# IllyaArtemchuk/Harmonies-Alphazero

Measured on AMD Instinct MI355X. Metric: self-play env-steps/sec + games/sec @4096 boards, 1/2/4/8 GPUs; bit-exact vs CPU, higher is better.
Workload: dtype u64; 1 GPU; config2: 4096 concurrent boards/GPU, reset + rule-driven play to game end (legal mask, step, chance draws, final scoring); one step = 256 hz_play launches of 4096 boards; boards_per_gpu=4096, parallelism=shard1

## Files before the change

### harmonies-alphazero_amd/csrc/hz_net.hip

```cpp
#include <hip/hip_runtime.h>

#include <atomic>
#include <cstdint>
#include <cstdlib>
#include <type_traits>

#include "../../include/hz_abi.h"
#include "hz_host.hpp"

using namespace hz_host;

namespace {

template <bool Res>
__global__ void __launch_bounds__(256) k_bias_act(float4 *__restrict__ x, const float4 *__restrict__ bias,
                                                  const float4 *__restrict__ res, int64_t n4, int32_t ch4) {
  int64_t i = (int64_t)blockIdx.x * 256 + threadIdx.x;
  if (i >= n4) return;
  float4 v = x[i];
  float4 b = bias[(int32_t)(i % ch4)];
  v.x = v.x + b.x;
  v.y = v.y + b.y;
  v.z = v.z + b.z;
  v.w = v.w + b.w;
// ... 706 lines not shown
    }
  }
  HZ_STAMP(7)
  HZ_STAMP_RT(9)
}
#undef HZ_X6_LOAD
#undef HZ_X6_STORE
#undef HZ_X6_SYNC

}

#ifndef HZ_KO
#define HZ_KO 0
#endif
namespace {
constexpr int kW4Stg = (kRows * 8 + 255) / 256;

template <int B, int E, class F>
__device__ __forceinline__ void static_for(F &&f) {
  if constexpr (B < E) {
    f(std::integral_constant<int, B>{});
    static_for<B + 1, E>(f);
  }
}
constexpr int x6_class_blocks(int h, int tap) {
  int k = 0;
  for (int rb = 0; rb < 9; rb++) k += (kX6ClassTaps[h][rb] >> tap) & 1;
  return k;
}

template <bool Block, bool Cf = false>
// ... 6 lines not shown
  if constexpr (NT) return __builtin_nontemporal_load((const f32x4 *)p);
  return *(const f32x4 *)p;
}
template <bool NT>
__device__ __forceinline__ float4 x6_ld4f(const float *p) {
  if constexpr (NT) {
    const f32x4 v = __builtin_nontemporal_load((const f32x4 *)p);
    return make_float4(v[0], v[1], v[2], v[3]);
  }
  return *(const float4 *)p;
}
template <bool Tower>
using X6In = std::conditional_t<Tower, const float *, const float *__restrict__>;
template <bool Tower>
using X6Out = std::conditional_t<Tower, float *, float *__restrict__>;
template <bool Block, bool Cf, bool Tower>
__device__ __forceinline__ void x6w4_body(X6In<Tower> x, const bf16x8 *__restrict__ wp,
                                          const float *__restrict__ bias, X6In<Tower> res,
                                          X6Out<Tower> out, int32_t batch, const int32_t *__restrict__ live,
                                          const bf16x8 *__restrict__ wp2, const float *__restrict__ bias2,
                                          float *__restrict__ tmp) {
  constexpr int NQ = 4, kRBT = 9, NCB = 4, NG = Block ? 8 : 4;
  constexpr int kZero = kCS * 35 * kX6Cell;
  constexpr int kBufT = kZero + kX6Zero;
  constexpr int kE = 2 * kBufT;
  static_assert(kZero % 256 == 0, "zero region 256-B aligned");
  constexpr int kDummyCell = kE + (kRows + 1) * 128;
  static_assert(kDummyCell + kX6Cell <= 160 * 1024, "buffers, E and the dummy cell fit the LDS");
  extern __shared__ float4 lds4[];
  char *lds = (char *)lds4;
  int t0 = threadIdx.x;
  if constexpr (Tower) asm volatile("" : "+v"(t0));
  __builtin_assume(t0 >= 0 && t0 < 256);
  const int t = t0, lane = t & 63, w = t >> 6, kg = lane >> 4, rh = w >> 1, chf = w & 1;
  const int s0 = blockIdx.x * kCS;
  if (live) batch = *live < batch ? *live : batch;
  if (s0 >= batch) return;
  const int ns = batch - s0 < kCS ? batch - s0 : kCS;
  HZ_STAMP(0)
  HZ_STAMP_RT(8)

  if (t < 2 * kX6Zero / 16) {
    const int b = t / (kX6Zero / 16), k = t - b * (kX6Zero / 16);
    *(float4 *)(lds + b * kBufT + kZero + 16 * k) = make_float4(0.f, 0.f, 0.f, 0.f);
  }
  f32x4 stg[kW4Stg];
  auto stage_f = [&](int it) {
    const int f = it * 256 + t;
    return f < kRows * 8 ? f : kRows * 8 - 1;
  };
  auto srow = [](int f) {
    const int r = f >> 3;
    return (r & ~3) | ((r & 1) << 1) | ((r >> 1) & 1);
// ... 2 lines not shown
  auto opaque_t = [&]() __attribute__((always_inline)) {
    int tt = t;
    if constexpr (Block) asm volatile("" : "+v"(tt));
    return tt;
  };
  auto stage_issue = [&](int q) __attribute__((always_inline)) {
    const int tt = opaque_t();
#pragma unroll
    for (int it = 0; it < kW4Stg; it++) {
      int f = it * 256 + tt;
      f = f < kRows * 8 ? f : kRows * 8 - 1;
      const int sc = s0 * 35 + srow(f);
      stg[it] = x6_ld4<Tower>(x + (size_t)(sc < last_row ? sc : last_row) * 128 + 4 * (f & 7) + 32 * q);
    }
  };
  constexpr int kTmpRows = 288;
  float *const tmpg = Block ? tmp + (size_t)blockIdx.x * 2 * kTmpRows * 32 : nullptr;
  auto stage_issue_e = [&]() __attribute__((always_inline)) {
    const int tt = opaque_t();
#pragma unroll
    for (int it = 0; it < kW4Stg; it++) {
      int f = it * 256 + tt;
      f = f < kRows * 8 ? f : kRows * 8 - 1;
      stg[it] = *(const f32x4 *)(lds + kE + 128 * srow(f) + 16 * (f & 7));
    }
  };
  auto stage_issue_tmp = [&](int half) __attribute__((always_inline)) {
    const int tt = opaque_t();
#pragma unroll
    for (int it = 0; it < kW4Stg; it++) {
      int f = it * 256 + tt;
      f = f < kRows * 8 ? f : kRows * 8 - 1;
      stg[it] = x6_ld4<Tower>(tmpg + half * kTmpRows * 32 + 32 * srow(f) + 4 * (f & 7));
    }
  };
  auto stage_put = [&](int it, int buf) {
    uint2 h, m, l;
    split4(stg[it], h, m, l);
    const int f = stage_f(it);
    char *d = lds + buf * kBufT + srow(f) * kX6Cell + 8 * (f & 7);
    *(uint2 *)d = h;
    *(uint2 *)(d + 64) = m;
    *(uint2 *)(d + 128) = l;
  };
  const int co0 = 64 * chf + (lane & 15);
  const bf16x8 *wl = wp + co0 * 4 + kg;
  const bf16x8 *wl2 = (Block ? wp2 : wp) + co0 * 4 + kg;
  auto bissue = [&](bf16x8(&dst)[3][NCB], int S) {
    S = S < 9 * NG ? S : 9 * NG - 1;
    const bf16x8 *w = wl;
    if constexpr (Block) {
      w = S < 9 * NQ ? wl : wl2;
      S = S < 9 * NQ ? S : S - 9 * NQ;
    }
    const int q2 = S / 9, t2 = S - 9 * q2;
#pragma unroll
    for (int p = 0; p < 3; p++)
#pragma unroll
      for (int cb = 0; cb < NCB; cb++) dst[p][cb] = w[((t2 * NQ + q2) * 3 + p) * 512 + 64 * cb];
  };
  int rtab[kRBT];
#pragma unroll
  for (int rb = 0; rb < kRBT; rb++) rtab[rb] = x6_tab<Block, Cf>()[rh * kRBT + rb][lane & 15];
  stage_issue(0);
  bf16x8 b[3][NCB], bn[3][NCB];
  bissue(b, 0);

  int cbase[kRBT];
  uint32_t valid[kRBT];
#pragma unroll
  for (int rb = 0; rb < kRBT; rb++) {
    const int r = rtab[rb] >= 0 ? rtab[rb] : 0;
    const int s = r / 35, cell = r - 35 * s, ch = cell / 7, cw = cell - 7 * ch;
    uint32_t v = 0;
#pragma unroll
    for (int tap = 0; tap < 9; tap++) {
      const int hh = ch + tap / 3 - 1, ww = cw + tap % 3 - 1;
      v |= (uint32_t)(hh >= 0 && hh < 5 && ww >= 0 && ww < 7) << tap;
// ... 9 lines not shown

  f32x4 acc[kRBT][NCB];
#pragma unroll
  for (int rb = 0; rb < kRBT; rb++)
#pragma unroll
    for (int cb = 0; cb < NCB; cb++) acc[rb][cb] = (f32x4){};
  HZ_STAMP(1)
#pragma unroll
  for (int it = 0; it < kW4Stg; it++) stage_put(it, 0);
  __syncthreads();
  HZ_STAMP(2)

  auto switch_convs = [&]() __attribute__((always_inline)) {
    float b1v[NCB];
#pragma unroll
    for (int cb = 0; cb < NCB; cb++) b1v[cb] = bias[64 * chf + 16 * cb + (lane & 15)];
    uint2 rows[kRBT];
#pragma unroll
    for (int rb = 0; rb < kRBT; rb++) rows[rb] = *(const uint2 *)&x6_tab<Block, Cf>()[rh * kRBT + rb][4 * kg];
    auto put_all = [&](auto chfc) __attribute__((always_inline)) {
      constexpr int C = decltype(chfc)::value;
      static_for<0, kRBT>([&](auto rbc) {
        constexpr int rb = decltype(rbc)::value;
        static_for<0, 4>([&](auto jc) {
          constexpr int j = decltype(jc)::value;
          const int r = (int)(int16_t)((j < 2 ? rows[rb].x : rows[rb].y) >> (16 * (j & 1)));
          const bool pad = r < 0;
          static_for<0, NCB>([&](auto cbc) {
            constexpr int cb = decltype(cbc)::value;
            float v = acc[rb][cb][j] + b1v[cb];
            v = v > 0.f ? v : 0.f;
            const int k = 16 * (cb & 1) + (lane & 15);
            if constexpr (cb >= 2) {
              tmpg[C * kTmpRows * 32 + (pad ? kRows : r) * 32 + k] = v;
            } else if constexpr (C == 0) {
              const uint32_t h = bf16_bits(v);
              const float r1 = v - bf16_value(h);
              const uint32_t m = bf16_bits(r1);
              const uint32_t l = bf16_bits(r1 - bf16_value(m));
              char *d = lds + (pad ? kDummyCell : r * kX6Cell) + 2 * k;
              *(unsigned short *)d = (unsigned short)h;
              *(unsigned short *)(d + 64) = (unsigned short)m;
              *(unsigned short *)(d + 128) = (unsigned short)l;
            } else {
              *(float *)(lds + kE + (pad ? kRows : r) * 128 + 4 * k) = v;
            }
          });
        });
        static_for<0, NCB>([&](auto cbc) { acc[rb][decltype(cbc)::value] = (f32x4){}; });
      });
    };
    if (chf == 0)
      put_all(std::integral_constant<int, 0>{});
    else
      put_all(std::integral_constant<int, 1>{});
    __syncthreads();
  };
  auto classed = [&](auto half) {
    constexpr int H = decltype(half)::value;
    auto aread = [&](bf16x8(&dst)[kRBT], const char *lb, auto tapc, int pa) {
      constexpr int tap = decltype(tapc)::value;
      static_for<0, kRBT>([&](auto rbc) {
        constexpr int rb = decltype(rbc)::value;
        if constexpr ((kX6ClassTaps[H][rb] >> tap) & 1) {
          constexpr int kNeg = 8 * kX6Cell;
          const int d = ((tap / 3 - 1) * 7 + (tap % 3 - 1)) * kX6Cell + kNeg + 64 * pa;
          if constexpr ((kX6ClassSel[H][rb] >> tap) & 1)
            dst[rb] = *(const bf16x8 *)(lb + aoff(rb, tap) + 64 * pa);
          else
            dst[rb] = *(const bf16x8 *)(lb - kNeg + cbase[rb] + d);
// ... 30 lines not shown
            if (tap == 0 && stage && !(HZ_KO & 1)) {
              if (Block && g == NQ + 1)
                stage_issue_e();
              else if (Block && g >= NQ)
                stage_issue_tmp(g == NQ + 2);
              else
                stage_issue(q + 1);
            }
          }
          if constexpr (HZ_KO & 2) {
            if (tap == 7 && pa == 1 && stage)
#pragma unroll
              for (int it = 0; it < kW4Stg; it++) asm volatile("" ::"v"(stg[it]));
          } else if constexpr (pa == 1 && !(HZ_KO & 1)) {
            if (stage) {
              if constexpr (tap >= 2 && tap <= 4) {
                stage_put(2 * (tap - 2), nb);
                stage_put(2 * (tap - 2) + 1, nb);
              } else if constexpr (tap >= 5 && tap <= 7) {
                stage_put(tap + 1, nb);
              }
            }
          }
#pragma unroll
          for (int pb = 0; pb < 3 - pa; pb++)
            static_for<0, kRBT>([&](auto rbc) {
              constexpr int rb = decltype(rbc)::value;
              if constexpr ((kX6ClassTaps[H][rb] >> tap) & 1) {
#pragma unroll
                for (int cb = 0; cb < NCB; cb++)
                  acc[rb][cb] = __builtin_amdgcn_mfma_f32_16x16x32_bf16(a[(HZ_KO & 32) ? 0 : cur][rb], b[pb][cb],
// ... 10 lines not shown
#pragma unroll
          for (int p = 0; p < 3; p++)
#pragma unroll
            for (int cb = 0; cb < NCB; cb++) b[p][cb] = bn[p][cb];
        }
      });
      __builtin_amdgcn_sched_barrier(0);
      if (sync) __syncthreads();
      if (g < NQ) {
        HZ_STAMP(3 + g)
      } else {
        HZ_STAMP(7 + g)
      }
    }
  };
  if (rh == 0)
    classed(std::integral_constant<int, 0>{});
  else
    classed(std::integral_constant<int, 1>{});

  constexpr int kTS = 20, kT = 6;
  static_assert(4 * kT * 16 * kTS * 4 <= kZero, "per-wave tiles fit in buffer 0");
  float *tile = (float *)lds + w * 16 * kTS * kT;
  const int trow = lane >> 2, tcol = 4 * (lane & 3);
  const int cow = 64 * chf + tcol;
  const int nrow = ns * 35;
  const size_t gbase = (size_t)s0 * 35 * 128;
  int erow[kRBT];
#pragma unroll
  for (int rb = 0; rb < kRBT; rb++) erow[rb] = x6_tab<Block, Cf>()[rh * kRBT + rb][lane >> 2];
  auto orow = [&](int rb) -> int {
    const int row = erow[rb];
    return row >= 0 && row < nrow ? row : -1;
  };
  const float *eres = Block ? x : res, *ebias = Block ? bias2 : bias;
  float4 rv[kRBT * NCB];
#pragma unroll
  for (int k = 0; k < kRBT * NCB; k++) {
    const int rb = k / NCB, cb = k % NCB;
    const int row = orow(rb);
    rv[k] = eres && row >= 0 && !(HZ_KO & 64) ? x6_ld4f<Tower>(eres + gbase + (size_t)row * 128 + cow + 16 * cb)
                                              : make_float4(0.f, 0.f, 0.f, 0.f);
  }
  if constexpr (Tower) asm volatile("" ::: "memory");
  float4 bv[NCB];
// ... 38 lines not shown
          if (never) *(float4 *)(out + gbase + (size_t)row * 128 + cow + 16 * cb) = v;
        } else
          *(float4 *)(out + gbase + (size_t)row * 128 + cow + 16 * cb) = v;
      }
    }
  }
  HZ_STAMP(7)
  HZ_STAMP_RT(9)
}
template <bool Block, bool Cf = false>
__global__ void __launch_bounds__(256, 1)
    k_conv3x3_x6w4(const float *__restrict__ x, const bf16x8 *__restrict__ wp, const float *__restrict__ bias,
                   const float *__restrict__ res, float *__restrict__ out, int32_t batch,
                   const int32_t *__restrict__ live, const bf16x8 *__restrict__ wp2,
                   const float *__restrict__ bias2, float *__restrict__ tmp) {
  x6w4_body<Block, Cf, false>(x, wp, bias, res, out, batch, live, wp2, bias2, tmp);
}
constexpr int kTowerMax = 16;
struct X6Tower {
  const bf16x8 *w1[kTowerMax], *w2[kTowerMax];
  const float *b1[kTowerMax], *b2[kTowerMax];
  int32_t nblk;
  int32_t stagger;
  int32_t round;
};
template <bool Cf>
__global__ void __launch_bounds__(256, 1)
    k_x6w4_tower(const float *__restrict__ x, float *out, int32_t batch, const int32_t *__restrict__ live,
                 float *__restrict__ tmp, X6Tower tw) {
  if (tw.stagger > 0 && (int)blockIdx.x < tw.round && ((blockIdx.x >> 3) & 1))
    for (int i = 0; i < tw.stagger; i++) __builtin_amdgcn_s_sleep(127);
#pragma unroll 1
  for (int k = 0; k < tw.nblk; k++) {
    x6w4_body<true, Cf, true>(k == 0 ? x : out, tw.w1[k], tw.b1[k], nullptr, out, batch, live, tw.w2[k], tw.b2[k],
                              tmp);
    asm volatile("s_waitcnt vmcnt(0)" ::: "memory");
    __syncthreads();
  }
}
}
#undef HZ_STAMP
#undef HZ_STAMP_RT

template <int NQ, bool Stem, int CS, int NCB, int Ord = 2>
static int launch_x6_cs(const float *x, const void *wpack6, const float *bias, const float *res, float *out,
                        int32_t batch, const int32_t *live, void *stream) {
  const size_t lds = 2 * (size_t)((CS * 35 * kX6Cell + 255) / 256 * 256 + kX6Zero);
  if (lds_opt_in<k_conv3x3_x6<NQ, Stem, CS, NCB, Ord>>(lds)) return 1;
  hipLaunchKernelGGL((k_conv3x3_x6<NQ, Stem, CS, NCB, Ord>), dim3((batch + CS - 1) / CS),
                     dim3((CS == 8 ? 2 : 1) * (8 / NCB) * 64), lds, (hipStream_t)stream, x, (const bf16x8 *)wpack6,
// ... 15 lines not shown
  static const bool v = env_pick("HZ_X6_W4", 0, 1);
  return v;
}

template <bool Block, bool Cf = false>
static int launch_x6w4(const float *x, const void *wpack6, const float *bias, const float *res, float *out,
                       int32_t batch, const int32_t *live, void *stream, const void *wpack6_2 = nullptr,
                       const float *bias2 = nullptr, float *tmp = nullptr) {
  const size_t lds = 2 * (size_t)(kCS * 35 * kX6Cell + kX6Zero) + (Block ? (size_t)(kRows + 1) * 128 + kX6Cell : 0);
  if (lds_opt_in<k_conv3x3_x6w4<Block, Cf>>(lds)) return 1;
  hipLaunchKernelGGL((k_conv3x3_x6w4<Block, Cf>), dim3((batch + kCS - 1) / kCS), dim3(256), lds, (hipStream_t)stream, x,
                     (const bf16x8 *)wpack6, bias, res, out, batch, live, (const bf16x8 *)wpack6_2, bias2, tmp);
  return hipGetLastError() == hipSuccess ? 0 : 1;
}

template <bool Cf>
static int launch_x6w4_tower(const float *x, float *out, float *tmp, const X6Tower &tw, int32_t batch,
                             const int32_t *live, void *stream) {
  const size_t lds = 2 * (size_t)(kCS * 35 * kX6Cell + kX6Zero) + (size_t)(kRows + 1) * 128 + kX6Cell;
  if (lds_opt_in<k_x6w4_tower<Cf>>(lds)) return 1;
  hipLaunchKernelGGL((k_x6w4_tower<Cf>), dim3((batch + kCS - 1) / kCS), dim3(256), lds, (hipStream_t)stream, x, out,
                     batch, live, tmp, tw);
  return hipGetLastError() == hipSuccess ? 0 : 1;
}

static Setting g_x6_block{"HZ_X6_BLOCK", 1};
static bool x6_block() { return g_x6_block.get() != 0; }

static Setting g_x6_blk_cf{"HZ_BLK_TABLE", 1};
static bool x6_blk_cf() { return g_x6_blk_cf.get() != 0; }

static bool stem_cs4() {
  static const bool v = env_pick("HZ_STEM_CS4", 0, 1);
  return v;
}
static bool x6_cs4() {
// ... 65 lines not shown
    int dev = 0, n = 0;
    if (hipGetDevice(&dev) == hipSuccess &&
        hipDeviceGetAttribute(&n, hipDeviceAttributeMultiprocessorCount, dev) == hipSuccess && n > 0)
      v = n;
    else
      v = 256;
    cus.store(v, std::memory_order_relaxed);
  }
  return v;
}
extern "C" int hz_tower_x6_set_stagger(int32_t units) {
  if (units < 0 || units > 1000) return -1;
  g_tower_stagger.set(units);
  return 0;
}
extern "C" int hz_tower_x6_blocks(const float *x, const void *const *w1, const float *const *b1,
                                  const void *const *w2, const float *const *b2, int32_t nblk, float *out,
                                  float *tmp, int32_t batch, const int32_t *live, void *stream) {
  if (!x || !w1 || !b1 || !w2 || !b2 || !out || !tmp || batch < 0 || nblk < 1 || nblk > kTowerMax) return -1;
  if (((uintptr_t)x | (uintptr_t)out | (uintptr_t)tmp) & 15) return -1;
  if (batch == 0) return 0;
  if (!hz_resblock_x6_fused(batch)) return -2;
  X6Tower tw{};
  for (int k = 0; k < nblk; k++) {
    if (!w1[k] || !b1[k] || !w2[k] || !b2[k] || (((uintptr_t)w1[k] | (uintptr_t)w2[k]) & 15)) return -1;
    tw.w1[k] = (const bf16x8 *)w1[k];
    tw.w2[k] = (const bf16x8 *)w2[k];
    tw.b1[k] = b1[k];
    tw.b2[k] = b2[k];
  }
  tw.nblk = nblk;
  tw.stagger = g_tower_stagger.get();
  tw.round = tower_round();
  return x6_blk_cf() ? launch_x6w4_tower<true>(x, out, tmp, tw, batch, live, stream)
                     : launch_x6w4_tower<false>(x, out, tmp, tw, batch, live, stream);
}

extern "C" int hz_resblock_x6_set_fused(int32_t on) {
  if (on != 0 && on != 1) return -1;
  g_x6_block.set(on);
  return 0;
}

extern "C" int hz_resblock_x6_set_table(int32_t cf) {
  if (cf != 0 && cf != 1) return -1;
  g_x6_blk_cf.set(cf);
  return 0;
}
// ... 14 lines not shown
namespace {
constexpr int kTRZero = 31 * 256;
constexpr int kTRChunk = kTRZero + 256 + 256;
constexpr int kTRBuf = 4 * kTRChunk;
constexpr int kTRLds = 2 * kTRBuf + 35 * 128 * 4;
constexpr int kTRMaxConv = 64;
constexpr int kTRConvW = 9 * 4 * 3 * 128 * 4;
constexpr int kTRAhead = 4;
static_assert(35 * kX6Cell <= kTRZero && kTRZero + 255 + 128 + 16 <= kTRChunk, "cells and zero region fit");
static_assert(36 % kTRAhead == 0, "the B ring's slots repeat every conv");

template <int Ord = 2>
__global__ void __launch_bounds__(512, 1)
    k_tower_x6_resident(const float *__restrict__ x0, const bf16x8 *__restrict__ wp,
                        const float *__restrict__ bias, float *__restrict__ out, int32_t nconv, int32_t batch,
                        const int32_t *__restrict__ live) {
  extern __shared__ float4 lds4[];
  char *lds = (char *)lds4;
  float *skip = (float *)(lds + 2 * kTRBuf);
  float *biasl = skip + 35 * 128;
  const int t = threadIdx.x, lane = t & 63, w = t >> 6, kg = lane >> 4;
  const int s = blockIdx.x;
  if (live) batch = *live < batch ? *live : batch;
  if (s >= batch) return;
  for (int i = t; i < nconv * 128; i += 512) biasl[i] = bias[i];

  if (t < 2 * 4 * 32) {
    const int c = t >> 5, k = t & 31;
    *(float4 *)(lds + c * kTRChunk + kTRZero + 16 * k) = make_float4(0.f, 0.f, 0.f, 0.f);
  }
  const float *xs = x0 + (size_t)s * 35 * 128;
  for (int f = t; f < 35 * 32; f += 512) {
    const f32x4 v = *(const f32x4 *)(xs + 4 * f);
    const int cell = f >> 5, part = f & 31;
    uint2 h, m, l;
    split4(v, h, m, l);
    char *d = lds + (part >> 3) * kTRChunk + cell * kX6Cell + 8 * (part & 7);
    *(uint2 *)d = h;
    if constexpr (Ord >= 1) *(uint2 *)(d + 64) = m;
// ... 93 lines not shown
  }
  static_assert(kTRAhead == 4, "the final wait names the ring's four slots");
  if constexpr (Ord == 2)
    asm volatile("s_waitcnt vmcnt(0)" ::: "memory");
  else if constexpr (Ord == 1)
    asm volatile("s_waitcnt vmcnt(0)"
                 : "+v"(bq[0][0]), "+v"(bq[0][1]), "+v"(bq[1][0]), "+v"(bq[1][1]), "+v"(bq[2][0]), "+v"(bq[2][1]),
                   "+v"(bq[3][0]), "+v"(bq[3][1])
                 :
                 : "memory");
  else
    asm volatile("s_waitcnt vmcnt(0)" : "+v"(bq[0][0]), "+v"(bq[1][0]), "+v"(bq[2][0]), "+v"(bq[3][0]) : : "memory");
}
}

extern "C" int hz_tower_x6_resident(const float *x0, const void *wpack6, const float *bias, float *out,
                                    int32_t nconv, int32_t batch, const int32_t *live, void *stream) {
  if (!x0 || !wpack6 || !bias || !out || batch < 0 || nconv < 2 || nconv > kTRMaxConv || (nconv & 1)) return -1;
  if (((uintptr_t)x0 | (uintptr_t)wpack6 | (uintptr_t)out) & 15) return -1;
  if (batch == 0) return 0;
  if (lds_opt_in<k_tower_x6_resident<>>(kTRLds + kTRMaxConv * 128 * 4)) return 1;
  hipLaunchKernelGGL(k_tower_x6_resident<>, dim3(batch), dim3(512), kTRLds + nconv * 128 * 4, (hipStream_t)stream, x0,
                     (const bf16x8 *)wpack6, bias, out, nconv, batch, live);
  return hipGetLastError() == hipSuccess ? 0 : 1;
}

template <int Ord>
static int launch_resident_xn(const float *x0, const void *wpack6, const float *bias, float *out, int32_t nconv,
                              int32_t batch, const int32_t *live, void *stream) {
  if (lds_opt_in<k_tower_x6_resident<Ord>>(kTRLds + kTRMaxConv * 128 * 4)) return 1;
  hipLaunchKernelGGL(k_tower_x6_resident<Ord>, dim3(batch), dim3(512), kTRLds + nconv * 128 * 4, (hipStream_t)stream,
                     x0, (const bf16x8 *)wpack6, bias, out, nconv, batch, live);
  return hipGetLastError() == hipSuccess ? 0 : 1;
}

extern "C" int hz_tower_xn_resident(const float *x0, const void *wpack6, const float *bias, float *out,
                                    int32_t nconv, int32_t batch, const int32_t *live, int32_t products,
                                    void *stream) {
  if (products != 1 && products != 3 && products != 6) return -1;
  if (products == 6) return hz_tower_x6_resident(x0, wpack6, bias, out, nconv, batch, live, stream);
  if (!x0 || !wpack6 || !bias || !out || batch < 0 || nconv < 2 || nconv > kTRMaxConv || (nconv & 1)) return -1;
  if (((uintptr_t)x0 | (uintptr_t)wpack6 | (uintptr_t)out) & 15) return -1;
  if (batch == 0) return 0;
  return products == 3 ? launch_resident_xn<1>(x0, wpack6, bias, out, nconv, batch, live, stream)
                       : launch_resident_xn<0>(x0, wpack6, bias, out, nconv, batch, live, stream);
}

// ... 791 lines not shown
```

### harmonies-alphazero_amd/hzamd/_native.py

```python
import ctypes
import os

import torch

PKG_DIR = os.path.dirname(os.path.dirname(os.path.abspath(__file__)))
LIB_PATH = os.environ.get("HZ_LIB") or os.path.join(PKG_DIR, "libhz.so")

_lib = None

_c = ctypes
_vp = ctypes.c_void_p
_SIGS = {
    "hz_env_create": ([_c.c_int32, _c.c_uint64, _vp], _vp),
    "hz_env_destroy": ([_vp], None),
    "hz_env_size": ([_vp], _c.c_int32),
    "hz_env_set_stream": ([_vp, _vp], _c.c_int),
    "hz_env_state_ptr": ([_vp], _vp),
    "hz_env_mt_ptr": ([_vp], _vp),
    "hz_env_mt_pos_ptr": ([_vp], _vp),
    "hz_env_stream_ptrs": ([_vp, _vp, _vp, _vp], _c.c_int),
    "hz_env_ply_ptr": ([_vp], _vp),
    "hz_env_seed_ptr": ([_vp], _vp),
    "hz_reset": ([_vp, _vp, _vp], _c.c_int),
    "hz_legal_mask": ([_vp, _vp, _vp], _c.c_int),
# ... 53 lines not shown
    "hz_bias_act": ([_vp, _vp, _vp, _c.c_int64, _c.c_int32, _vp], _c.c_int),
    "hz_conv3x3_bias_act": ([_vp, _vp, _vp, _vp, _vp, _c.c_int32, _vp, _vp], _c.c_int),
    "hz_heads": ([_vp, _vp, _vp, _vp, _vp, _vp, _c.c_int32, _vp, _vp], _c.c_int),
    "hz_heads_fc": ([_vp] * 13 + [_c.c_int32, _vp, _vp], _c.c_int),
    "hz_conv3x3_x6_bias_act": ([_vp, _vp, _vp, _vp, _vp, _c.c_int32, _vp, _vp], _c.c_int),
    "hz_conv3x3_xn_bias_act": ([_vp, _vp, _vp, _vp, _vp, _c.c_int32, _vp, _c.c_int32, _vp], _c.c_int),
    "hz_tower_xn_resident": ([_vp, _vp, _vp, _vp, _c.c_int32, _c.c_int32, _vp, _c.c_int32, _vp], _c.c_int),
    "hz_stem3x3_x6_bias_act": ([_vp, _vp, _vp, _vp, _c.c_int32, _vp, _vp], _c.c_int),
    "hz_resblock_x6_bias_act": ([_vp, _vp, _vp, _vp, _vp, _vp, _vp, _c.c_int32, _vp, _vp], _c.c_int),
    "hz_resblock_x6_fused": ([_c.c_int32], _c.c_int32),
    "hz_resblock_x6_set_fused": ([_c.c_int32], _c.c_int),
    "hz_resblock_x6_set_table": ([_c.c_int32], _c.c_int),
    "hz_tower_x6_set_stagger": ([_c.c_int32], _c.c_int),
    "hz_tower_x6_blocks": ([_vp, _vp, _vp, _vp, _vp, _c.c_int32, _vp, _vp, _c.c_int32, _vp, _vp], _c.c_int),
    "hz_tower_x6_resident": ([_vp, _vp, _vp, _vp, _c.c_int32, _c.c_int32, _vp, _vp], _c.c_int),
    "hz_tower_x6_split": ([_vp, _vp, _vp, _vp, _vp, _vp, _c.c_int32, _c.c_int32, _vp, _vp], _c.c_int),
    "hz_tower_x6_split_max_batch": ([], _c.c_int32),
    "hz_tower_x6_split_set_limit": ([_c.c_int32], _c.c_int),
    "hz_conv3x3_x6g_bias_act": ([_vp, _vp, _vp, _vp, _vp, _c.c_int32, _c.c_int32, _c.c_int32, _vp, _c.c_int32,
                                 _c.c_int32, _vp], _c.c_int),
    "hz_stem3x3_x6g_bias_act": ([_vp, _vp, _vp, _vp, _c.c_int32, _c.c_int32, _vp, _c.c_int32, _vp], _c.c_int),
    "hz_heads_fc_g": ([_vp] * 13 + [_c.c_int32] * 5 + [_vp, _vp], _c.c_int),
    "hz_stem3x3_bias_act": ([_vp, _vp, _vp, _vp, _c.c_int32, _vp, _vp], _c.c_int),
    "hz_version": ([], _c.c_char_p),
}


class NativeError(RuntimeError):
    pass

# ... 41 lines not shown
```

### harmonies-alphazero_amd/hzamd/infer.py

```python
import ctypes
import os

import torch
import torch.nn.functional as F
from torch import nn

from ._native import NativeError, lib


def pack_conv3x3(w):
    co, ci = w.shape[0], w.shape[1]
    return w.permute(2, 3, 1, 0).reshape(9, ci // 16, 16, co).permute(0, 1, 3, 2).contiguous()


def split3_bf16(w):
    w = w.float()
    h = w.to(torch.bfloat16)
    r = w - h.float()
    m = r.to(torch.bfloat16)
    lo = (r - m.float()).to(torch.bfloat16)
    return torch.stack((h, m, lo))


def pack_conv3x3_x6(w):
# ... 189 lines not shown

def _resblock_x6(x, p1, b1, p2, b2, live=None):
    if not (x.is_cuda and x.dtype == torch.float32 and x.is_contiguous(memory_format=torch.channels_last)
            and x.shape[1:] == (128, 5, 7)):
        raise NativeError("hz_resblock_x6_bias_act needs a CUDA fp32 channels_last [B,128,5,7] activation")
    out = torch.empty_like(x, memory_format=torch.channels_last)
    tmp = torch.empty_like(x, memory_format=torch.channels_last)
    rc = lib().hz_resblock_x6_bias_act(x.data_ptr(), p1.data_ptr(), b1.data_ptr(), p2.data_ptr(), b2.data_ptr(),
                                       out.data_ptr(), tmp.data_ptr(), x.shape[0], _live_ptr(live),
                                       torch.cuda.current_stream(x.device).cuda_stream)
    if rc != 0:
        raise NativeError(f"hz_resblock_x6_bias_act failed ({rc})")
    return out


def _tower_blocks_x6(x, ptrs, nblk, live=None):
    out = torch.empty_like(x, memory_format=torch.channels_last)
    tmp = torch.empty_like(x, memory_format=torch.channels_last)
    w1, b1, w2, b2 = ptrs
    rc = lib().hz_tower_x6_blocks(x.data_ptr(), w1, b1, w2, b2, nblk, out.data_ptr(), tmp.data_ptr(), x.shape[0],
                                  _live_ptr(live), torch.cuda.current_stream(x.device).cuda_stream)
    if rc == -2:
        return None
    if rc != 0:
        raise NativeError(f"hz_tower_x6_blocks failed ({rc})")
    return out


def pack_stem_x6(w):
    co = w.shape[0]
    w64 = torch.zeros(co, 64, 3, 3, dtype=w.dtype, device=w.device)
    w64[:, :w.shape[1]] = w
    w64[:, 38] = w64[:, 39] = w[:, 37]
    pl = split3_bf16(w64)
    pl[2, :, 38] = 0
    pl[1:, :, 39] = 0
# ... 151 lines not shown
def _fold(conv, bn):
    inv = torch.rsqrt(bn.running_var.double() + bn.eps) * bn.weight.double()
    w = (conv.weight.double() * inv.view(-1, 1, 1, 1)).float()
    b0 = conv.bias.double() if conv.bias is not None else torch.zeros_like(inv)
    b = ((b0 - bn.running_mean.double()) * inv + bn.bias.double()).float()
    return w.contiguous(memory_format=torch.channels_last), b.contiguous()


class FoldedNet(nn.Module):

    TOWER_MFMA = ("x6", "x3", "x1", "f32")
    TOWER_PRODUCTS = {"x6": 6, "x3": 3, "x1": 1}
    resident_max = int(os.environ.get("HZ_RESIDENT_MAX", "896"))
    split_max = int(os.environ.get("HZ_SPLIT_MAX", "32"))
    tower_loop = int(os.environ.get("HZ_TOWER_LOOP", "1"))
    wide_spg = 0

    def __init__(self, net, epilogue=None, native_conv=True, tower=None, fused_head=True):
        super().__init__()
        if tower is None:
            tower = os.environ.get("HZ_TOWER", "x6")
        if tower not in self.TOWER_MFMA:
            raise ValueError(f"tower must be one of {self.TOWER_MFMA}, not {tower!r}")
        self.src = net
        self.tower = tower
        self.fused_head = fused_head
        self.epilogue = epilogue or _bias_act
        self.native_conv = native_conv and epilogue is None
        self.refresh()

# ... 112 lines not shown
            xs = _tower_split(x, *self.resident, live)
        if xs is not None:
            x = xs
        elif products in (3, 1) and self.packed is not None:
            if self.resident is not None and B <= self.resident_max:
                x = _tower_resident(x, *self.resident, live, products)
            else:
                for ((_, b1), (_, b2)), (p1, p2) in zip(self.blocks, self.packed):
                    y = _conv3x3_xn_act(x, p1, b1, None, live, products)
                    x = _conv3x3_xn_act(y, p2, b2, x, live, products)
        elif self.resident is not None and B <= max(self.resident_max, min(self.split_max, 32)):
            x = _tower_resident(x, *self.resident, live)
        elif self.packed is not None and self.tower == "x6":
            xt = None
            if self.tower_loop and len(self.blocks) <= 16:
                xt = _tower_blocks_x6(x, self._tw_ptrs, len(self.blocks), live)
            if xt is not None:
                x = xt
            else:
                for ((_, b1), (_, b2)), (p1, p2) in zip(self.blocks, self.packed):
                    x = _resblock_x6(x, p1, b1, p2, b2, live)
        elif self.packed is not None:
            for ((_, b1), (_, b2)), (p1, p2) in zip(self.blocks, self.packed):
                y = _conv3x3_act(x, p1, b1, None, live)
                x = _conv3x3_act(y, p2, b2, x, live)
        else:
            for (w1, b1), (w2, b2) in self.blocks:
                y = ep(_nhwc(F.conv2d(x, w1, None, padding=1)), b1)
                x = ep(_nhwc(F.conv2d(y, w2, None, padding=1)), b2, x)
        if self.fc is not None:
            lo, pr, v = _heads_fc(x, glob, *self.heads, self.fc, live=live, logits=not probs, probs=probs)
# ... 16 lines not shown
```

### include/hz_abi.h

```cpp
#ifndef HZ_ABI_H
#define HZ_ABI_H
#include <stdint.h>

#ifdef __cplusplus
extern "C" {
#endif

enum {
  HZ_ST_OK = 0,
  HZ_ST_BAD_PILE = 1,
  HZ_ST_BAD_FORMAT = 2,
  HZ_ST_NOT_IN_HAND = 3,
  HZ_ST_ILLEGAL_STACK = 4,
  HZ_ST_BAD_PHASE = 5,
  HZ_ST_BAD_ACTION = 6,
  HZ_ST_NOOP = 7
};

typedef struct hz_env hz_env;

hz_env *hz_env_create(int32_t n_boards, uint64_t seed_base, void *stream);
void hz_env_destroy(hz_env *env);
int32_t hz_env_size(const hz_env *env);
int hz_env_set_stream(hz_env *env, void *stream);
// ... 98 lines not shown
int hz_conv3x3_x6_bias_act(const float *x, const void *wpack6, const float *bias, const float *res, float *out,
                           int32_t batch, const int32_t *live, void *stream);

int hz_conv3x3_xn_bias_act(const float *x, const void *wpack6, const float *bias, const float *res,
                           float *out, int32_t batch, const int32_t *live, int32_t products, void *stream);

int hz_resblock_x6_bias_act(const float *x, const void *w1, const float *b1, const void *w2, const float *b2,
                            float *out, float *tmp, int32_t batch, const int32_t *live, void *stream);
int32_t hz_resblock_x6_fused(int32_t batch);
int hz_resblock_x6_set_fused(int32_t on);
int hz_resblock_x6_set_table(int32_t cf);
int hz_tower_x6_blocks(const float *x, const void *const *w1, const float *const *b1, const void *const *w2,
                       const float *const *b2, int32_t nblk, float *out, float *tmp, int32_t batch,
                       const int32_t *live, void *stream);
int hz_tower_x6_set_stagger(int32_t units);

int hz_stem3x3_bias_act(const float *board, const float *wpack, const float *bias, float *out, int32_t batch,
                        const int32_t *live, void *stream);
int hz_stem3x3_x6_bias_act(const float *board, const void *wpack6, const float *bias, float *out, int32_t batch,
                           const int32_t *live, void *stream);
int hz_tower_x6_resident(const float *x0, const void *wpack6, const float *bias, float *out, int32_t nconv,
                         int32_t batch, const int32_t *live, void *stream);
int hz_tower_xn_resident(const float *x0, const void *wpack6, const float *bias, float *out, int32_t nconv,
                         int32_t batch, const int32_t *live, int32_t products, void *stream);
int hz_tower_x6_split(const float *x0, const void *wpack6, const float *bias, float *out, float *xch, uint32_t *sync,
                      int32_t nconv, int32_t batch, const int32_t *live, void *stream);

int32_t hz_tower_x6_split_max_batch(void);
int hz_tower_x6_split_set_limit(int32_t groups);

// ... 23 lines not shown
```

Baseline: 23.87 billion env-steps/s.

## Add 4-state tower units and live-gated resident/looped tower dispatch

Templates the fused residual-block body on states per workgroup and adds a 4-state variant. A per-launch plan splits small live batches into 4-state units so more CUs get work. Also adds a gate: when the live count is at or below a threshold, the resident per-state tower kernel runs; above it, the looped block kernel runs. Both are launched and each exits early on device based on the live count. This adds code complexity and an extra launch in exchange for better CU utilisation at small live batches.

```diff
diff --git a/harmonies-alphazero_amd/csrc/hz_net.hip b/harmonies-alphazero_amd/csrc/hz_net.hip
--- a/harmonies-alphazero_amd/csrc/hz_net.hip
+++ b/harmonies-alphazero_amd/csrc/hz_net.hip
@@ -744,7 +744,6 @@
 #define HZ_KO 0
 #endif
 namespace {
-constexpr int kW4Stg = (kRows * 8 + 255) / 256;
 
 template <int B, int E, class F>
 __device__ __forceinline__ void static_for(F &&f) {
@@ -781,14 +780,16 @@
 using X6In = std::conditional_t<Tower, const float *, const float *__restrict__>;
 template <bool Tower>
 using X6Out = std::conditional_t<Tower, float *, float *__restrict__>;
-template <bool Block, bool Cf, bool Tower>
+template <bool Block, bool Cf, bool Tower, int CS = kCS>
 __device__ __forceinline__ void x6w4_body(X6In<Tower> x, const bf16x8 *__restrict__ wp,
                                           const float *__restrict__ bias, X6In<Tower> res,
                                           X6Out<Tower> out, int32_t batch, const int32_t *__restrict__ live,
                                           const bf16x8 *__restrict__ wp2, const float *__restrict__ bias2,
-                                          float *__restrict__ tmp) {
-  constexpr int NQ = 4, kRBT = 9, NCB = 4, NG = Block ? 8 : 4;
-  constexpr int kZero = kCS * 35 * kX6Cell;
+                                          float *__restrict__ tmpg, const int s0) {
+  static_assert(CS == 8 || (CS == 4 && Block), "8 states, or 4 in the fused block");
+  constexpr int NQ = 4, kRBT = 9, NCB = CS == 8 ? 4 : 2, NG = Block ? 8 : 4;
+  constexpr int kRows = CS * 35, kW4Stg = (kRows * 8 + 255) / 256;
+  constexpr int kZero = (kRows * kX6Cell + 255) / 256 * 256;
   constexpr int kBufT = kZero + kX6Zero;
   constexpr int kE = 2 * kBufT;
   static_assert(kZero % 256 == 0, "zero region 256-B aligned");
@@ -799,11 +800,14 @@
   int t0 = threadIdx.x;
   if constexpr (Tower) asm volatile("" : "+v"(t0));
   __builtin_assume(t0 >= 0 && t0 < 256);
-  const int t = t0, lane = t & 63, w = t >> 6, kg = lane >> 4, rh = w >> 1, chf = w & 1;
-  const int s0 = blockIdx.x * kCS;
+  const int t = t0, lane = t & 63, w = t >> 6, kg = lane >> 4, rh = CS == 8 ? w >> 1 : 0, chf = CS == 8 ? w & 1 : w;
   if (live) batch = *live < batch ? *live : batch;
   if (s0 >= batch) return;
-  const int ns = batch - s0 < kCS ? batch - s0 : kCS;
+  const int ns = batch - s0 < CS ? batch - s0 : CS;
+  auto tab_row = [&](int rb) -> const int16_t * {
+    if constexpr (CS == 4) return kX6C4Row[rb];
+    return x6_tab<Block, Cf>()[rh * kRBT + rb];
+  };
   HZ_STAMP(0)
   HZ_STAMP_RT(8)
 
@@ -836,8 +840,7 @@
       stg[it] = x6_ld4<Tower>(x + (size_t)(sc < last_row ? sc : last_row) * 128 + 4 * (f & 7) + 32 * q);
     }
   };
-  constexpr int kTmpRows = 288;
-  float *const tmpg = Block ? tmp + (size_t)blockIdx.x * 2 * kTmpRows * 32 : nullptr;
+  constexpr int kTmpRows = CS == 8 ? 288 : 144;
   auto stage_issue_e = [&]() __attribute__((always_inline)) {
     const int tt = opaque_t();
 #pragma unroll
@@ -865,7 +868,7 @@
     *(uint2 *)(d + 64) = m;
     *(uint2 *)(d + 128) = l;
   };
-  const int co0 = 64 * chf + (lane & 15);
+  const int co0 = 16 * NCB * chf + (lane & 15);
   const bf16x8 *wl = wp + co0 * 4 + kg;
   const bf16x8 *wl2 = (Block ? wp2 : wp) + co0 * 4 + kg;
   auto bissue = [&](bf16x8(&dst)[3][NCB], int S) {
@@ -883,7 +886,10 @@
   };
   int rtab[kRBT];
 #pragma unroll
-  for (int rb = 0; rb < kRBT; rb++) rtab[rb] = x6_tab<Block, Cf>()[rh * kRBT + rb][lane & 15];
+  for (int rb = 0; rb < kRBT; rb++) {
+    rtab[rb] = tab_row(rb)[lane & 15];
+    if constexpr (CS == 4) rtab[rb] = rtab[rb] >= 0 ? rtab[rb] : tab_row(rb)[0];
+  }
   stage_issue(0);
   bf16x8 b[3][NCB], bn[3][NCB];
   bissue(b, 0);
@@ -923,12 +929,12 @@
   auto switch_convs = [&]() __attribute__((always_inline)) {
     float b1v[NCB];
 #pragma unroll
-    for (int cb = 0; cb < NCB; cb++) b1v[cb] = bias[64 * chf + 16 * cb + (lane & 15)];
+    for (int cb = 0; cb < NCB; cb++) b1v[cb] = bias[16 * NCB * chf + 16 * cb + (lane & 15)];
     uint2 rows[kRBT];
 #pragma unroll
-    for (int rb = 0; rb < kRBT; rb++) rows[rb] = *(const uint2 *)&x6_tab<Block, Cf>()[rh * kRBT + rb][4 * kg];
+    for (int rb = 0; rb < kRBT; rb++) rows[rb] = *(const uint2 *)&tab_row(rb)[4 * kg];
     auto put_all = [&](auto chfc) __attribute__((always_inline)) {
-      constexpr int C = decltype(chfc)::value;
+      constexpr int W = decltype(chfc)::value;
       static_for<0, kRBT>([&](auto rbc) {
         constexpr int rb = decltype(rbc)::value;
         static_for<0, 4>([&](auto jc) {
@@ -939,10 +945,11 @@
             constexpr int cb = decltype(cbc)::value;
             float v = acc[rb][cb][j] + b1v[cb];
             v = v > 0.f ? v : 0.f;
+            constexpr int Q = CS == 8 ? 2 * W + (cb >> 1) : W;
             const int k = 16 * (cb & 1) + (lane & 15);
-            if constexpr (cb >= 2) {
-              tmpg[C * kTmpRows * 32 + (pad ? kRows : r) * 32 + k] = v;
-            } else if constexpr (C == 0) {
+            if constexpr (Q & 1) {
+              tmpg[(Q >> 1) * kTmpRows * 32 + (pad ? kRows : r) * 32 + k] = v;
+            } else if constexpr (Q == 0) {
               const uint32_t h = bf16_bits(v);
               const float r1 = v - bf16_value(h);
               const uint32_t m = bf16_bits(r1);
@@ -959,10 +966,16 @@
         static_for<0, NCB>([&](auto cbc) { acc[rb][decltype(cbc)::value] = (f32x4){}; });
       });
     };
-    if (chf == 0)
-      put_all(std::integral_constant<int, 0>{});
-    else
-      put_all(std::integral_constant<int, 1>{});
+    if constexpr (CS == 8) {
+      if (chf == 0)
+        put_all(std::integral_constant<int, 0>{});
+      else
+        put_all(std::integral_constant<int, 1>{});
+    } else {
+      static_for<0, 4>([&](auto wc) {
+        if (chf == decltype(wc)::value) put_all(wc);
+      });
+    }
     __syncthreads();
   };
   auto classed = [&](auto half) {
@@ -1023,7 +1036,9 @@
               for (int it = 0; it < kW4Stg; it++) asm volatile("" ::"v"(stg[it]));
           } else if constexpr (pa == 1 && !(HZ_KO & 1)) {
             if (stage) {
-              if constexpr (tap >= 2 && tap <= 4) {
+              if constexpr (CS == 4) {
+                if constexpr (tap >= 2 && tap <= 6) stage_put(tap - 2, nb);
+              } else if constexpr (tap >= 2 && tap <= 4) {
                 stage_put(2 * (tap - 2), nb);
                 stage_put(2 * (tap - 2) + 1, nb);
               } else if constexpr (tap >= 5 && tap <= 7) {
@@ -1064,21 +1079,23 @@
       }
     }
   };
-  if (rh == 0)
+  if constexpr (CS == 4)
+    classed(std::integral_constant<int, 2>{});
+  else if (rh == 0)
     classed(std::integral_constant<int, 0>{});
   else
     classed(std::integral_constant<int, 1>{});
 
   constexpr int kTS = 20, kT = 6;
-  static_assert(4 * kT * 16 * kTS * 4 <= kZero, "per-wave tiles fit in buffer 0");
+  static_assert(4 * kT * 16 * kTS * 4 <= kZero && (kRBT * NCB) % kT == 0, "per-wave tiles fit in buffer 0");
   float *tile = (float *)lds + w * 16 * kTS * kT;
   const int trow = lane >> 2, tcol = 4 * (lane & 3);
-  const int cow = 64 * chf + tcol;
+  const int cow = 16 * NCB * chf + tcol;
   const int nrow = ns * 35;
   const size_t gbase = (size_t)s0 * 35 * 128;
   int erow[kRBT];
 #pragma unroll
-  for (int rb = 0; rb < kRBT; rb++) erow[rb] = x6_tab<Block, Cf>()[rh * kRBT + rb][lane >> 2];
+  for (int rb = 0; rb < kRBT; rb++) erow[rb] = tab_row(rb)[lane >> 2];
   auto orow = [&](int rb) -> int {
     const int row = erow[rb];
     return row >= 0 && row < nrow ? row : -1;
@@ -1147,7 +1164,8 @@
                    const float *__restrict__ res, float *__restrict__ out, int32_t batch,
                    const int32_t *__restrict__ live, const bf16x8 *__restrict__ wp2,
                    const float *__restrict__ bias2, float *__restrict__ tmp) {
-  x6w4_body<Block, Cf, false>(x, wp, bias, res, out, batch, live, wp2, bias2, tmp);
+  x6w4_body<Block, Cf, false>(x, wp, bias, res, out, batch, live, wp2, bias2,
+                              Block ? tmp + (size_t)blockIdx.x * 2 * 288 * 32 : nullptr, blockIdx.x * kCS);
 }
 constexpr int kTowerMax = 16;
 struct X6Tower {
@@ -1156,17 +1174,44 @@
   int32_t nblk;
   int32_t stagger;
   int32_t round;
+  int32_t plan;
+  int32_t gate;
 };
+constexpr int kTmp8 = 2 * 288 * 32, kTmp4 = 2 * 144 * 32;
+struct X6Unit {
+  int32_t cs, s0;
+  size_t tmp;
+};
+__device__ __forceinline__ X6Unit x6_plan(int32_t L, int32_t C, int32_t i) {
+  if (C > 0 && L <= 4 * C) return {4, 4 * i, (size_t)i * kTmp4};
+  if (C > 0 && L > 8 * C && L <= 12 * C && i >= C) return {4, 8 * C + 4 * (i - C), (size_t)C * kTmp8 + (size_t)(i - C) * kTmp4};
+  return {8, 8 * i, (size_t)i * kTmp8};
+}
 template <bool Cf>
 __global__ void __launch_bounds__(256, 1)
     k_x6w4_tower(const float *__restrict__ x, float *out, int32_t batch, const int32_t *__restrict__ live,
                  float *__restrict__ tmp, X6Tower tw) {
+  int32_t L = batch;
+  if (live) L = *live < batch ? *live : batch;
+  if (L <= tw.gate) return;
+  const X6Unit u = x6_plan(L, tw.plan, blockIdx.x);
+  if (u.s0 >= L) return;
   if (tw.stagger > 0 && (int)blockIdx.x < tw.round && ((blockIdx.x >> 3) & 1))
     for (int i = 0; i < tw.stagger; i++) __builtin_amdgcn_s_sleep(127);
+  if (u.cs == 4) {
+#pragma unroll 1
+    for (int k = 0; k < tw.nblk; k++) {
+      x6w4_body<true, Cf, true, 4>(k == 0 ? x : out, tw.w1[k], tw.b1[k], nullptr, out, batch, live, tw.w2[k],
+                                   tw.b2[k], tmp + u.tmp, u.s0);
+      asm volatile("s_waitcnt vmcnt(0)" ::: "memory");
+      __syncthreads();
+    }
+    return;
+  }
 #pragma unroll 1
   for (int k = 0; k < tw.nblk; k++) {
     x6w4_body<true, Cf, true>(k == 0 ? x : out, tw.w1[k], tw.b1[k], nullptr, out, batch, live, tw.w2[k], tw.b2[k],
-                              tmp);
+                              tmp + u.tmp, u.s0);
     asm volatile("s_waitcnt vmcnt(0)" ::: "memory");
     __syncthreads();
   }
@@ -1212,12 +1257,30 @@
   return hipGetLastError() == hipSuccess ? 0 : 1;
 }
 
+static int32_t tower_grid(int32_t batch, int32_t plan) {
+  const int64_t B = batch, C = plan;
+  int64_t g = (B + 7) / 8;
+  if (C > 0) {
+    g = std::max(g, (std::min(B, 4 * C) + 3) / 4);
+    if (B > 8 * C) g = std::max(g, C + (std::min(B, 12 * C) - 8 * C + 3) / 4);
+  }
+  return (int32_t)g;
+}
+static int64_t tower_tmp_floats(int32_t batch, int32_t plan) {
+  const int64_t B = batch, C = plan;
+  int64_t n = (B + 7) / 8 * kTmp8;
+  if (C > 0) {
+    n = std::max(n, (std::min(B, 4 * C) + 3) / 4 * kTmp4);
+    if (B > 8 * C) n = std::max(n, C * kTmp8 + (std::min(B, 12 * C) - 8 * C + 3) / 4 * kTmp4);
+  }
+  return n;
+}
 template <bool Cf>
 static int launch_x6w4_tower(const float *x, float *out, float *tmp, const X6Tower &tw, int32_t batch,
                              const int32_t *live, void *stream) {
   const size_t lds = 2 * (size_t)(kCS * 35 * kX6Cell + kX6Zero) + (size_t)(kRows + 1) * 128 + kX6Cell;
   if (lds_opt_in<k_x6w4_tower<Cf>>(lds)) return 1;
-  hipLaunchKernelGGL((k_x6w4_tower<Cf>), dim3((batch + kCS - 1) / kCS), dim3(256), lds, (hipStream_t)stream, x, out,
+  hipLaunchKernelGGL((k_x6w4_tower<Cf>), dim3(tower_grid(batch, tw.plan)), dim3(256), lds, (hipStream_t)stream, x, out,
                      batch, live, tmp, tw);
   return hipGetLastError() == hipSuccess ? 0 : 1;
 }
@@ -1313,9 +1376,28 @@
   g_tower_stagger.set(units);
   return 0;
 }
+static Setting g_tower_plan{"HZ_TOWER_PLAN", 1};
+static Setting g_tower_plan_round{"HZ_TOWER_PLAN_ROUND", 0};
+extern "C" int hz_tower_x6_set_plan(int32_t on) {
+  if (on != 0 && on != 1) return -1;
+  g_tower_plan.set(on);
+  return 0;
+}
+extern "C" int hz_tower_x6_set_plan_round(int32_t cus) {
+  if (cus < 0 || cus > 4096) return -1;
+  g_tower_plan_round.set(cus);
+  return 0;
+}
 extern "C" int hz_tower_x6_blocks(const float *x, const void *const *w1, const float *const *b1,
                                   const void *const *w2, const float *const *b2, int32_t nblk, float *out,
                                   float *tmp, int32_t batch, const int32_t *live, void *stream) {
+  return hz_tower_x6_blocks_gated(x, w1, b1, w2, b2, nblk, out, tmp, batch, live, 0, stream);
+}
+extern "C" int hz_tower_x6_blocks_gated(const float *x, const void *const *w1, const float *const *b1,
+                                        const void *const *w2, const float *const *b2, int32_t nblk, float *out,
+                                        float *tmp, int32_t batch, const int32_t *live, int32_t gate,
+                                        void *stream) {
+  if (gate < 0) return -1;
   if (!x || !w1 || !b1 || !w2 || !b2 || !out || !tmp || batch < 0 || nblk < 1 || nblk > kTowerMax) return -1;
   if (((uintptr_t)x | (uintptr_t)out | (uintptr_t)tmp) & 15) return -1;
   if (batch == 0) return 0;
@@ -1331,6 +1413,9 @@
   tw.nblk = nblk;
   tw.stagger = g_tower_stagger.get();
   tw.round = tower_round();
+  tw.gate = gate;
+  tw.plan = g_tower_plan.get() ? (g_tower_plan_round.get() ? g_tower_plan_round.get() : tw.round) : 0;
+  if (tower_tmp_floats(batch, tw.plan) > (int64_t)batch * 35 * 128) tw.plan = 0;
   return x6_blk_cf() ? launch_x6w4_tower<true>(x, out, tmp, tw, batch, live, stream)
                      : launch_x6w4_tower<false>(x, out, tmp, tw, batch, live, stream);
 }
@@ -1375,7 +1460,7 @@
 __global__ void __launch_bounds__(512, 1)
     k_tower_x6_resident(const float *__restrict__ x0, const bf16x8 *__restrict__ wp,
                         const float *__restrict__ bias, float *__restrict__ out, int32_t nconv, int32_t batch,
-                        const int32_t *__restrict__ live) {
+                        const int32_t *__restrict__ live, int32_t gate) {
   extern __shared__ float4 lds4[];
   char *lds = (char *)lds4;
   float *skip = (float *)(lds + 2 * kTRBuf);
@@ -1383,7 +1468,7 @@
   const int t = threadIdx.x, lane = t & 63, w = t >> 6, kg = lane >> 4;
   const int s = blockIdx.x;
   if (live) batch = *live < batch ? *live : batch;
-  if (s >= batch) return;
+  if (s >= batch || (gate > 0 && batch > gate)) return;
   for (int i = t; i < nconv * 128; i += 512) biasl[i] = bias[i];
 
   if (t < 2 * 4 * 32) {
@@ -1507,14 +1592,27 @@
 }
 }
 
+static int resident_x6(const float *x0, const void *wpack6, const float *bias, float *out, int32_t nconv,
+                       int32_t batch, const int32_t *live, int32_t gate, void *stream);
 extern "C" int hz_tower_x6_resident(const float *x0, const void *wpack6, const float *bias, float *out,
                                     int32_t nconv, int32_t batch, const int32_t *live, void *stream) {
+  return resident_x6(x0, wpack6, bias, out, nconv, batch, live, 0, stream);
+}
+extern "C" int hz_tower_x6_resident_gated(const float *x0, const void *wpack6, const float *bias, float *out,
+                                          int32_t nconv, int32_t batch, const int32_t *live, int32_t gate,
+                                          void *stream) {
+  if (gate < 1) return -1;
+  return resident_x6(x0, wpack6, bias, out, nconv, batch, live, gate, stream);
+}
+static int resident_x6(const float *x0, const void *wpack6, const float *bias, float *out, int32_t nconv,
+                       int32_t batch, const int32_t *live, int32_t gate, void *stream) {
   if (!x0 || !wpack6 || !bias || !out || batch < 0 || nconv < 2 || nconv > kTRMaxConv || (nconv & 1)) return -1;
   if (((uintptr_t)x0 | (uintptr_t)wpack6 | (uintptr_t)out) & 15) return -1;
   if (batch == 0) return 0;
   if (lds_opt_in<k_tower_x6_resident<>>(kTRLds + kTRMaxConv * 128 * 4)) return 1;
-  hipLaunchKernelGGL(k_tower_x6_resident<>, dim3(batch), dim3(512), kTRLds + nconv * 128 * 4, (hipStream_t)stream, x0,
-                     (const bf16x8 *)wpack6, bias, out, nconv, batch, live);
+  const int32_t grid = gate > 0 && gate < batch ? gate : batch;
+  hipLaunchKernelGGL(k_tower_x6_resident<>, dim3(grid), dim3(512), kTRLds + nconv * 128 * 4, (hipStream_t)stream, x0,
+                     (const bf16x8 *)wpack6, bias, out, nconv, batch, live, gate);
   return hipGetLastError() == hipSuccess ? 0 : 1;
 }
 
@@ -1523,7 +1621,7 @@
                               int32_t batch, const int32_t *live, void *stream) {
   if (lds_opt_in<k_tower_x6_resident<Ord>>(kTRLds + kTRMaxConv * 128 * 4)) return 1;
   hipLaunchKernelGGL(k_tower_x6_resident<Ord>, dim3(batch), dim3(512), kTRLds + nconv * 128 * 4, (hipStream_t)stream,
-                     x0, (const bf16x8 *)wpack6, bias, out, nconv, batch, live);
+                     x0, (const bf16x8 *)wpack6, bias, out, nconv, batch, live, 0);
   return hipGetLastError() == hipSuccess ? 0 : 1;
 }
 
diff --git a/harmonies-alphazero_amd/hzamd/_native.py b/harmonies-alphazero_amd/hzamd/_native.py
--- a/harmonies-alphazero_amd/hzamd/_native.py
+++ b/harmonies-alphazero_amd/hzamd/_native.py
@@ -91,6 +91,11 @@
     "hz_tower_x6_set_stagger": ([_c.c_int32], _c.c_int),
     "hz_tower_x6_blocks": ([_vp, _vp, _vp, _vp, _vp, _c.c_int32, _vp, _vp, _c.c_int32, _vp, _vp], _c.c_int),
     "hz_tower_x6_resident": ([_vp, _vp, _vp, _vp, _c.c_int32, _c.c_int32, _vp, _vp], _c.c_int),
+    "hz_tower_x6_set_plan": ([_c.c_int32], _c.c_int),
+    "hz_tower_x6_set_plan_round": ([_c.c_int32], _c.c_int),
+    "hz_tower_x6_blocks_gated": ([_vp, _vp, _vp, _vp, _vp, _c.c_int32, _vp, _vp, _c.c_int32, _vp, _c.c_int32, _vp],
+                                 _c.c_int),
+    "hz_tower_x6_resident_gated": ([_vp, _vp, _vp, _vp, _c.c_int32, _c.c_int32, _vp, _c.c_int32, _vp], _c.c_int),
     "hz_tower_x6_split": ([_vp, _vp, _vp, _vp, _vp, _vp, _c.c_int32, _c.c_int32, _vp, _vp], _c.c_int),
     "hz_tower_x6_split_max_batch": ([], _c.c_int32),
     "hz_tower_x6_split_set_limit": ([_c.c_int32], _c.c_int),
diff --git a/harmonies-alphazero_amd/hzamd/infer.py b/harmonies-alphazero_amd/hzamd/infer.py
--- a/harmonies-alphazero_amd/hzamd/infer.py
+++ b/harmonies-alphazero_amd/hzamd/infer.py
@@ -227,12 +227,24 @@
     return out
 
 
-def _tower_blocks_x6(x, ptrs, nblk, live=None):
+def _tower_blocks_x6(x, ptrs, nblk, live=None, resident=None, gate=0):
     out = torch.empty_like(x, memory_format=torch.channels_last)
     tmp = torch.empty_like(x, memory_format=torch.channels_last)
     w1, b1, w2, b2 = ptrs
-    rc = lib().hz_tower_x6_blocks(x.data_ptr(), w1, b1, w2, b2, nblk, out.data_ptr(), tmp.data_ptr(), x.shape[0],
-                                  _live_ptr(live), torch.cuda.current_stream(x.device).cuda_stream)
+    stream = torch.cuda.current_stream(x.device).cuda_stream
+    if resident is None or live is None or gate <= 0:
+        rc = lib().hz_tower_x6_blocks(x.data_ptr(), w1, b1, w2, b2, nblk, out.data_ptr(), tmp.data_ptr(), x.shape[0],
+                                      _live_ptr(live), stream)
+    else:
+        if not lib().hz_resblock_x6_fused(x.shape[0]):
+            return None
+        allw, allb = resident
+        rc = lib().hz_tower_x6_resident_gated(x.data_ptr(), allw.data_ptr(), allb.data_ptr(), out.data_ptr(),
+                                              allw.shape[0], x.shape[0], _live_ptr(live), gate, stream)
+        if rc != 0:
+            raise NativeError(f"hz_tower_x6_resident_gated failed ({rc})")
+        rc = lib().hz_tower_x6_blocks_gated(x.data_ptr(), w1, b1, w2, b2, nblk, out.data_ptr(), tmp.data_ptr(),
+                                            x.shape[0], _live_ptr(live), gate, stream)
     if rc == -2:
         return None
     if rc != 0:
@@ -414,6 +426,7 @@
     resident_max = int(os.environ.get("HZ_RESIDENT_MAX", "896"))
     split_max = int(os.environ.get("HZ_SPLIT_MAX", "32"))
     tower_loop = int(os.environ.get("HZ_TOWER_LOOP", "1"))
+    tower_gate = int(os.environ.get("HZ_TOWER_GATE", "512"))
     wide_spg = 0
 
     def __init__(self, net, epilogue=None, native_conv=True, tower=None, fused_head=True):
@@ -556,7 +569,9 @@
         elif self.packed is not None and self.tower == "x6":
             xt = None
             if self.tower_loop and len(self.blocks) <= 16:
-                xt = _tower_blocks_x6(x, self._tw_ptrs, len(self.blocks), live)
+                gated = live is not None and self.resident is not None and hasattr(lib(), "hz_tower_x6_blocks_gated")
+                xt = _tower_blocks_x6(x, self._tw_ptrs, len(self.blocks), live, self.resident if gated else None,
+                                      self.tower_gate)
             if xt is not None:
                 x = xt
             else:
diff --git a/include/hz_abi.h b/include/hz_abi.h
--- a/include/hz_abi.h
+++ b/include/hz_abi.h
@@ -136,6 +136,13 @@
                        const float *const *b2, int32_t nblk, float *out, float *tmp, int32_t batch,
                        const int32_t *live, void *stream);
 int hz_tower_x6_set_stagger(int32_t units);
+int hz_tower_x6_set_plan(int32_t on);
+int hz_tower_x6_set_plan_round(int32_t cus);
+int hz_tower_x6_blocks_gated(const float *x, const void *const *w1, const float *const *b1, const void *const *w2,
+                             const float *const *b2, int32_t nblk, float *out, float *tmp, int32_t batch,
+                             const int32_t *live, int32_t gate, void *stream);
+int hz_tower_x6_resident_gated(const float *x0, const void *wpack6, const float *bias, float *out, int32_t nconv,
+                               int32_t batch, const int32_t *live, int32_t gate, void *stream);
 
 int hz_stem3x3_bias_act(const float *board, const float *wpack, const float *bias, float *out, int32_t batch,
                         const int32_t *live, void *stream);
```

After: 23.86 billion env-steps/s. Within noise of the previous version (-0.0%).
